# liangheming/simple_pose

Measured on AMD Instinct MI355X. Metric: images/sec fwd+decode, ResNet50-DConv 256x192 bs=128, higher is better.
Workload: dtype f32; 1 GPU; ResNet50-DConv 256x192 bs=128 per GPU, fp32 forward (NCHW in -> heat maps) + GaussTaylor decode, eval-mode BN, conditioned random weights; images_per_gpu=128, global_batch=128, parallelism=replicas x1 (no collective), ranks=1 process(es), one per GPU, launch=stream launches, tile_table=profiles/r06_dconv_f32_tiles.json, batches_in_flight=2, decode=in line, HSA_ENABLE_IPC_MODE_LEGACY=0

## Files before the change

include/simple_pose_hip.h:

```cpp
#ifndef SIMPLE_POSE_HIP_H
#define SIMPLE_POSE_HIP_H

#include <stdint.h>

#ifdef __cplusplus
extern "C" {
#endif

#define SP_OK 0
#define SP_EINVAL (-1)
#define SP_ELAUNCH (-2)

#define SP_ABI_VERSION 36

#define SP_CONV_RELU 0x1u
#define SP_CONV_OUT_NCHW 0x2u
#define SP_CONV_PIXEL_SHUFFLE 0x4u
#define SP_CONV_OUT_F32 0x10u
#define SP_CONV_BN_Y_MASK 0x20u
#define SP_CONV_BF16 0x8u
#define SP_CONV_HARDSWISH 0x40u
#define SP_CONV_OUT_SLICE 0x80u

typedef struct sp_conv_desc {
// ... 1 lines not shown
    int32_t grid_h, grid_w;
    int32_t c_out;
    int32_t n_pad;
    int32_t taps_h, taps_w;
    int32_t k_pad;
    int32_t stride;
    int32_t dy0, dy_step, dx0, dx_step;
    int32_t out_h, out_w, out_c;
    int32_t oy_mul, oy_add, ox_mul, ox_add;
    int32_t phases_y, phases_x;
    uint32_t flags;
    int32_t tile_m, tile_n;
    int32_t stride_x;
    int32_t kernel;
    int32_t c_in_group;
} sp_conv_desc;

#define SP_CONV_KERNEL_IGEMM 0
#define SP_CONV_KERNEL_RING 1
#define SP_CONV_KERNEL_RING_LW 3
#define SP_CONV_KERNEL_RING_LW4 4
#define SP_CONV_KERNEL_PW 2

int sp_abi_version(void);
const char* sp_last_error(void);


int sp_nchw_to_nhwc4(const float* x_nchw, float* y_nhwc4, int batch, int channels, int h, int w, void* stream);

int sp_conv2d_fwd(const sp_conv_desc* desc, const void* x, const void* w_packed, const float* scale,
                  const float* shift, const void* residual, void* y, void* stream);

int sp_conv_set_tap_skip(int on);

int sp_conv3x3_direct_ok(const sp_conv_desc* desc);
int sp_conv3x3_direct(const sp_conv_desc* desc, const void* x, const void* w_packed, const float* scale, const float* shift,
                      const void* residual, void* y, void* stream);

int sp_basic_block_c32_ok(const sp_conv_desc* desc);
int sp_basic_block_c32(const sp_conv_desc* desc, const void* x, const void* w1_packed, const float* scale1, const float* shift1,
                       const void* w2_packed, const float* scale2, const float* shift2, void* y, void* stream);

int sp_basic_block_c64_ok(const sp_conv_desc* desc);
int sp_basic_block_c64(const sp_conv_desc* desc, const void* x, const void* w1_packed, const float* scale1, const float* shift1,
                       const void* w2_packed, const float* scale2, const float* shift2, void* y, void* stream);

int sp_dual_pw_bf16_ok(int64_t rows, int c_main, int c_short, int c_out);
int sp_dual_pw_f32_ok(int64_t rows, int c_main, int c_short, int c_out);
int sp_dual_pw_f32(const float* a_main, const float* w_main_packed, const float* scale_main, const float* shift_main, const float* a_short,
                   const float* w_short_packed, const float* scale_short, const float* shift_short, float* y, int64_t rows, int c_main, int c_short,
                   int c_out, int relu, void* stream);
int sp_dual_pw_bf16(const void* a_main, const void* w_main_packed, const float* scale_main, const float* shift_main, const void* a_short,
                    const void* w_short_packed, const float* scale_short, const float* shift_short, void* y, int64_t rows, int c_main, int c_short,
                    int c_out, int relu, void* stream);
int sp_pw_chain_f32_ok(int64_t rows, int c_mid, int c_out, int c_next);
int sp_pw_chain_f32(const float* t, const float* w3_packed, const float* scale3, const float* shift3, const float* residual, float* y,
                    const float* w1_packed, const float* scale1, const float* shift1, float* t_next, int64_t rows, int c_mid, int c_out, int c_next,
                    void* stream);
int sp_bottleneck_c64_ok(const sp_conv_desc* desc);
int sp_bottleneck_c64(const sp_conv_desc* desc, const void* x, const void* w1_packed, const float* scale1, const float* shift1,
                      const void* w2_packed, const float* scale2, const float* shift2, const void* w3_packed, const float* scale3,
                      const float* shift3, void* y, void* stream);

int sp_stem7_pool_ok(int batch, int h, int w);
int sp_stem7_pool(const float* x, const void* w_packed, int k_pad, const float* scale, const float* shift, void* y, int bf16,
                  int batch, int h, int w, void* stream);
// ... 547 lines not shown
```

simple_pose_amd/_lib.py:

```python
from __future__ import annotations

import ctypes
import os
from ctypes import c_double, c_float, c_int, c_int32, c_int64, c_uint32, c_void_p

from .build import LIB_PATH as _DEFAULT_LIB_PATH

LIB_PATH = os.environ.get("SIMPLE_POSE_HIP_LIB", _DEFAULT_LIB_PATH)

SP_CONV_RELU = 0x1
SP_CONV_OUT_NCHW = 0x2
SP_CONV_PIXEL_SHUFFLE = 0x4
SP_CONV_BF16 = 0x8
SP_CONV_OUT_F32 = 0x10
SP_CONV_BN_Y_MASK = 0x20
SP_CONV_HARDSWISH = 0x40
SP_CONV_OUT_SLICE = 0x80
SP_LETTERBOX_FOCUS, SP_LETTERBOX_U8 = 0, 1
SP_YOLO_NMS_MAX_CANDIDATES, SP_YOLO_NMS_MAX_DET = 32768, 1024
SP_COCO_MAX_JOINTS, SP_COCO_MAX_GT_PER_IMAGE, SP_COCO_MAX_DT_PER_IMAGE, SP_COCO_MAX_DETS = 64, 128, 2048, 32
SP_COCO_DT_XY_F64, SP_COCO_DT_SCORE_F64, SP_COCO_GT_CROWD, SP_COCO_GT_IGNORE = 1, 2, 1, 2
CONV_TILES =((128, 128), (64, 128), (128, 64), (64, 64), (256, 64), (128, 32))
ABI_VERSION = 36
SP_CONV_KERNEL_IGEMM, SP_CONV_KERNEL_RING, SP_CONV_KERNEL_PW, SP_CONV_KERNEL_RING_LW, SP_CONV_KERNEL_RING_LW4 = 0, 1, 2, 3, 4
# ... 104 lines not shown


SP_HEAT_ALPHA_CONSTANT, SP_HEAT_ALPHA_VALUE = 0, 1
SP_HEAT_ALPHAS = {"constant": SP_HEAT_ALPHA_CONSTANT, "value": SP_HEAT_ALPHA_VALUE}
SP_HEAT_MAX_MAP = 256

class TileRef(ctypes.Structure):
    _fields_ = [("data", ctypes.c_uint64), ("h", c_int32), ("w", c_int32), ("pitch", c_int32), ("new_h", c_int32), ("new_w", c_int32),
                ("top", c_int32), ("left", c_int32), ("ratio", c_float), ("x0", c_int32), ("y0", c_int32), ("image", c_int32),
                ("slot", c_int32)]


SP_TILE_MAX_TILES, SP_TILE_MAX_PASSES = 64, 65


class YuvRef(ctypes.Structure):
    _fields_ = [("y", ctypes.c_uint64), ("u", ctypes.c_uint64), ("v", ctypes.c_uint64), ("bgr", ctypes.c_uint64), ("h", c_int32), ("w", c_int32),
                ("pitch_y", c_int32), ("pitch_c", c_int32), ("pitch_bgr", c_int32), ("format", c_int32), ("matrix", c_int32), ("range", c_int32)]


assert ctypes.sizeof(YuvRef) == 64
SP_YUV_NV12, SP_YUV_I420 = 0, 1
SP_YUV_BT601, SP_YUV_BT709 = 0, 1
SP_YUV_LIMITED, SP_YUV_FULL = 0, 1
SP_TILE_IOU, SP_TILE_IOS = 0, 1

_P = c_void_p
SYMBOLS = {
    "sp_abi_version": (c_int, []),
    "sp_last_error": (ctypes.c_char_p, []),
    "sp_nchw_to_nhwc4": (c_int, [_P, _P, c_int, c_int, c_int, c_int, _P]),
    "sp_conv2d_fwd": (c_int, [ctypes.POINTER(ConvDesc), _P, _P, _P, _P, _P, _P, _P]),
    "sp_conv_set_tap_skip": (c_int, [c_int]),
    "sp_conv2d_ring_ok": (c_int, [ctypes.POINTER(ConvDesc)]),
    "sp_conv2d_kernel_name": (c_int, [ctypes.POINTER(ConvDesc), c_int, c_int, ctypes.c_char_p, c_int]),
    "sp_conv2d_default_tile": (c_int, [ctypes.POINTER(ConvDesc), ctypes.POINTER(c_int), ctypes.POINTER(c_int)]),
    "sp_maxpool3x3s2_nhwc": (c_int, [_P, _P, c_int, c_int, c_int, c_int, _P]),
    "sp_pixel_shuffle2_nhwc": (c_int, [_P, _P, c_int, c_int, c_int, c_int, _P]),
    "sp_global_avg_pool_nhwc": (c_int, [_P, _P, c_int, c_int, c_int, _P]),
    "sp_se_gate_add_relu_nhwc": (c_int, [_P, _P, _P, _P, c_int, c_int, c_int, _P]),
    "sp_upsample_add_nhwc": (c_int, [_P, _P, _P, c_int, c_int, c_int, c_int, c_int, c_int, _P]),
    "sp_nchw_to_nhwc8_bf16": (c_int, [_P, _P, c_int, c_int, c_int, c_int, _P]),
    "sp_maxpool3x3s2_nhwc_bf16": (c_int, [_P, _P, c_int, c_int, c_int, c_int, _P]),
    "sp_pixel_shuffle2_nhwc_bf16": (c_int, [_P, _P, c_int, c_int, c_int, c_int, _P]),
    "sp_upsample_add_nhwc_bf16": (c_int, [_P, _P, _P, c_int, c_int, c_int, c_int, c_int, c_int, _P]),
    "sp_global_avg_pool_nhwc_bf16": (c_int, [_P, _P, c_int, c_int, c_int, _P]),
    "sp_se_gate_add_relu_nhwc_bf16": (c_int, [_P, _P, _P, _P, c_int, c_int, c_int, _P]),
    "sp_heat_map_to_axis": (c_int, [_P, c_int, c_int, c_int, c_int, _P, _P, _P]),
    "sp_decode_gauss_taylor": (c_int, [_P, _P, c_int, c_int, c_int, c_int, c_int, _P, _P, _P]),
    "sp_decode_basic": (c_int, [_P, _P, c_int, c_int, c_int, c_int, _P, _P, _P]),
    "sp_heat_map_acc": (c_int, [_P, _P, _P, c_int, c_int, c_int, c_int, c_float, c_float, _P, _P]),
    "sp_u8hwc_bgr_to_nchw_f32": (c_int, [_P, _P, c_int, c_int, c_int, ctypes.POINTER(c_float), _P]),
    "sp_encode_gauss_refine": (c_int, [_P, c_int, c_int, c_int, c_int, c_float, _P, _P, _P]),
    "sp_encode_gauss_basic": (c_int, [_P, c_int, c_int, c_int, c_int, c_float, c_int, _P, _P, _P]),
    "sp_bn_train_stats_nhwc": (c_int, [_P, c_int, c_int64, c_int, c_float, c_float, _P, _P, _P, _P, _P, _P]),
    "sp_bn_apply_maxpool_nhwc": (c_int, [_P, c_int, _P, _P, _P, _P, _P, _P, c_int, c_int, c_int, c_int, _P]),
    "sp_bn_maxpool_bwd_nhwc": (c_int, [_P, c_int, _P, _P, _P, _P, _P, _P, c_int, c_int, c_int, c_int, _P, _P, _P, _P, _P]),
    "sp_bn_apply_nhwc": (c_int, [_P, c_int, _P, _P, _P, _P, _P, _P, c_int64, c_int, c_int, _P, _P]),
    "sp_bn_train_partial_nhwc": (c_int, [_P, c_int, c_int64, c_int, _P, _P, _P]),
    "sp_bn_train_finalize": (c_int, [_P, c_int64, c_int, c_float, c_float, _P, _P, _P, _P, _P]),
    "sp_bn_apply_sums_nhwc": (c_int, [_P, c_int, _P, c_int64, c_float, c_float, _P, _P, _P, _P, c_int64, c_int, c_int, _P, _P, _P, _P, _P]),
    "sp_bn_bwd_sums_from_conv2": (c_int, [_P, _P, c_int, c_int, c_int, _P, _P, _P, _P, _P]),
    "sp_bn_train_bwd_reduce_nhwc": (c_int, [_P, c_int, _P, _P, _P, _P, c_int64, c_int, _P, _P, _P, _P]),
    "sp_bn_train_bwd_apply_nhwc": (c_int, [_P, c_int, _P, _P, _P, _P, _P, _P, _P, c_int64, c_int64, c_int, _P, _P, c_int, _P]),
    "sp_bn_train_bwd_nhwc": (c_int, [_P, c_int, _P, _P, _P, _P, _P, c_int64, c_int, _P, _P, _P, _P, c_int, _P, _P]),
    "sp_channel_sum_nchw": (c_int, [_P, c_int, c_int, c_int, _P, _P]),
# ... 132 lines not shown
    "sp_yuv420_to_bgr_images_u8c3": (c_int, [_P, c_int, c_int, c_int, _P]),
    "sp_bgr_to_yuv420_images_u8c3": (c_int, [_P, c_int, c_int, c_int, _P]),
    "sp_yuv420_wide_path": (c_int, [_P, _P, _P, _P, c_int, c_int, c_int, c_int]),
}

_lib = None


def lib():
    global _lib
    if _lib is None:
        if not os.path.isfile(LIB_PATH):
            raise HipLibraryError(
                f"{LIB_PATH} is missing: build it with `python -m simple_pose_amd.build` (hipcc, gfx950). "
                "simple_pose_amd has no CPU/torch fallback.")
        import torch

        handle = ctypes.CDLL(LIB_PATH)
        for name, (res, args) in SYMBOLS.items():
            fn = getattr(handle, name)
            fn.restype, fn.argtypes = res, args
        if handle.sp_abi_version() != ABI_VERSION:
            raise HipLibraryError(f"ABI mismatch: library {handle.sp_abi_version()} vs binding {ABI_VERSION}")
        _lib = handle
    return _lib


def conv_kernel_name(desc, has_residual: bool = False, variant: int = 0) -> str:
    buf = ctypes.create_string_buffer(256)
    check(lib().sp_conv2d_kernel_name(desc, int(has_residual), variant, buf, 256), "sp_conv2d_kernel_name")
    return buf.value.decode()


def check(rc: int, what: str = ""):
    if rc != 0:
        msg = lib().sp_last_error().decode("utf-8", "replace")
        err = HipLibraryError(f"{what or 'libsimple_pose_hip'} failed (code {rc}): {msg}")
        err.code = rc
        raise err


def ptr(t):
    return None if t is None else t.data_ptr()


import threading

_pin = threading.local()


def _device_index(device) -> int:
    if device is None:
        import torch
        return torch.cuda.current_device()
    if isinstance(device, int):
        return device
    idx = getattr(device, "index", None)
    if idx is None:
        import torch
        return torch.cuda.current_device()
    return idx


def pin_stream(pin):
    prev = getattr(_pin, "value", None)
    _pin.value = pin
# ... 35 lines not shown
```

simple_pose_amd/csrc/conv_igemm.hip:

```cpp
#include "sp_common.h"
#include <stdlib.h>
#include <type_traits>

#ifdef SP_DIAG
__device__ unsigned long long sp_dbg[4096 * 4 * 12];
extern "C" int sp_debug_read(unsigned long long* dst, int n) {
    return (int)hipMemcpyFromSymbol(dst, HIP_SYMBOL(sp_dbg), sizeof(unsigned long long) * n, 0, hipMemcpyDeviceToHost);
}
extern "C" int sp_debug_clear() {
    static unsigned long long z[4096 * 4 * 12];
    return (int)hipMemcpyToSymbol(HIP_SYMBOL(sp_dbg), z, sizeof(z), 0, hipMemcpyHostToDevice);
}
#define SP_STAMP_ALWAYS(var)                                                                \
    unsigned long long var;                                                                 \
    __builtin_amdgcn_sched_barrier(0);                                                      \
    asm volatile("s_memtime %0\n\ts_waitcnt lgkmcnt(0)" : "=s"(var)::"memory");           \
    __builtin_amdgcn_sched_barrier(0);
#ifdef SP_DIAG_LIGHT
#define SP_STAMP(var) unsigned long long var = 0;
#else
#define SP_STAMP(var) SP_STAMP_ALWAYS(var)
#endif
#else
#define SP_STAMP(var)
// ... 30 lines not shown
    const float* binvstd;
    int bz_bytes;
    const void* bz2;
    const float* bmean2;
    const float* binvstd2;
    float* stats_q2;
    struct PhaseGeo { const void* w; int taps_h, taps_w, k_pad, dy0, dx0, oy_add, ox_add, pad_; } ph[4];
    int ph_n;
    int c_in_g;
    const float* abn_mean;
    const float* abn_invstd;
    const float* abn_gamma;
    const float* abn_beta;
    void* abn_y;
    unsigned char* abn_mask;
    int batch;
};

constexpr int BK = 32;

__device__ __forceinline__ float hardswish(float v) {
#pragma clang fp contract(off)
    return v * fminf(fmaxf(v + 3.f, 0.f), 6.f) / 6.f;
}

__device__ __forceinline__ int swz(int row, int chunk) { return row * BK + ((chunk ^ ((row >> 1) & 7)) << 2); }


__device__ __forceinline__ float abn_elem(float v, float mu, float is, float g, float b) {
#pragma clang fp contract(off)
    return (v - mu) * is * g + b;
}

template <int BM, int BN, int WR, int WC, bool UNIFORM_TAP, bool BF16, bool OUT16, bool STATS, bool DEEP, bool BSTATS, bool ABN, bool SKIP = false>
__device__ __forceinline__ void conv_igemm_body(const ConvArgs& p) {
    static_assert(!ABN || (UNIFORM_TAP && BF16 && OUT16 && STATS && !DEEP && !BSTATS), "ABN: the bf16 train-mode forward of a 1x1 conv");
    static_assert(!SKIP || (UNIFORM_TAP && !BF16 && !OUT16 && !STATS && !DEEP && !BSTATS && !ABN), "SKIP: the plain fp32 inference instantiation");
    constexpr int ES = BF16 ? 2 : 4;
    constexpr int EPC = 16 / ES;
    constexpr int BKE = 128 / ES;
    constexpr int ESO = OUT16 ? 2 : 4;
    static_assert(BF16 || !OUT16, "bf16 output needs bf16 inputs");
    static_assert(WR * WC == 4, "4 waves per workgroup");
    constexpr int WM = BM / WR, WN = BN / WC;
    constexpr int TM = WM / 32, TN = WN / 32;
    constexpr int A_CH = BM / 32, B_CH = BN / 32;
    static_assert(TM >= 1 && TN >= 1, "wave tile must hold at least one 32x32 MFMA tile");

#ifdef SP_DIAG
    SP_STAMP_ALWAYS(t_entry)
#endif
#ifdef SP_DIAG
    unsigned long long rt_entry;
    asm volatile("s_memrealtime %0\n\ts_waitcnt lgkmcnt(0)" : "=s"(rt_entry)::"memory");
#endif
    extern __shared__ __attribute__((aligned(16))) float smem[];
    float* As = smem;
    float* Bs = smem + 2 * BM * BK;
    int* rowtab = reinterpret_cast<int*>(smem + 2 * (BM + BN) * BK);

    const int tid = threadIdx.x;
    const int lane = tid & 63;
    const int wave = __builtin_amdgcn_readfirstlane(tid >> 6);
    const int wr = wave / WC, wc = wave % WC;

    const int nwg = p.tiles_m * p.tiles_n;
    int t;
    {
        const int orig = blockIdx.x;
        const int xcd = orig & 7, q = nwg >> 3, r = nwg & 7;
        t = (xcd < r ? xcd * (q + 1) : r * (q + 1) + (xcd - r) * q) + (orig >> 3);
    }
    const int tn = t % p.tiles_n, tm = t / p.tiles_n;
    int tm_rows = tm;
    if constexpr (SKIP) {
        const int Q = p.tiles_m >> 3, R = p.tiles_m & 7;
        int x, i;
        if (tm < R * (Q + 1)) { x = tm / (Q + 1); i = tm - x * (Q + 1); }
        else { const int u = tm - R * (Q + 1); x = u / Q; i = u - x * Q; x += R; }
        tm_rows = i * 8 + x;
    }
    const int m0 = tm_rows * BM, n0 = tn * BN;

    const int phase = blockIdx.y;
    const int py = phase / p.phases_x, px = phase % p.phases_x;
    int dy0 = p.dy0 + py, dx0 = p.dx0 + px;
    int oy_add = p.oy_add + py, ox_add = p.ox_add + px;
    int taps_h = p.taps_h, taps_w = p.taps_w, k_pad = p.k_pad, w_bytes = p.w_bytes;
    const char* __restrict__ wp = reinterpret_cast<const char*>(p.w) + (size_t)phase * p.n_pad * p.k_pad * ES;
    if (p.ph_n) {
        const ConvArgs::PhaseGeo& g = p.ph[phase];
        dy0 = g.dy0; dx0 = g.dx0; oy_add = g.oy_add; ox_add = g.ox_add;
// ... 206 lines not shown
            acc[i][n] = __builtin_amdgcn_mfma_f32_32x32x2f32(fa[slot][i][s], fb[slot][n][s], acc[i][n], 0, 0, 0);
    };
#define SP_SB() __builtin_amdgcn_sched_barrier(0)

    tile_taps(0);
#pragma unroll
    for (int i = 0; i < A_CH; ++i) load_a(i, I0{});
#pragma unroll
    for (int i = 0; i < B_CH; ++i) load_b(i, I0{});
    if constexpr (PF > 1) {
        auto request = [&](auto j_tag) {
            constexpr int J = decltype(j_tag)::value;
            if (J < nk) {
                tile_taps(J);
#pragma unroll
                for (int i = 0; i < A_CH; ++i) load_a(i, j_tag);
#pragma unroll
                for (int i = 0; i < B_CH; ++i) load_b(i, j_tag);
            }
        };
        request(std::integral_constant<int, 1>{});
        if constexpr (PF == 4) { request(std::integral_constant<int, 2>{}); request(std::integral_constant<int, 3>{}); }
    }
#pragma unroll
    for (int o = 0; o < NOPS; ++o) store_piece(0, o, I0{});
    __syncthreads();
    read_frags(As + (wr * WM) * BK, Bs + (wc * WN) * BK, 0, 0);

#ifdef SP_DIAG
    unsigned long long dg[8] = {0, 0, 0, 0, 0, 0, 0, 0};
#endif
    auto k_tile = [&](int kt, auto more_tag) {
        constexpr bool MORE = decltype(more_tag)::value;
        const int cur = kt & 1;
        const float* a = As + cur * BM * BK + (wr * WM) * BK;
        const float* b = Bs + cur * BN * BK + (wc * WN) * BK;
        const float* an = As + (cur ^ 1) * BM * BK + (wr * WM) * BK;
        const float* bn = Bs + (cur ^ 1) * BN * BK + (wc * WN) * BK;
        SP_STAMP(s0)
        read_frags(a, b, 1, 1);
        if (MORE) tile_taps(kt + 1);
        SP_SB();
#pragma unroll
        for (int q = 0; q < NM; ++q) {
            mfma_q(0, q);
            if (MORE) {
#pragma unroll
                for (int o = (q * NOPS) / NM; o < ((q + 1) * NOPS) / NM; ++o) {
                    if (o < A_CH) load_a(o, I0{}); else load_b(o - A_CH, I0{});
                }
            }
            SP_SB();
        }
        SP_STAMP(s1)
        read_frags(a, b, 2, 0);
#pragma unroll
        for (int q = 0; q < NM; ++q) mfma_q(1, q);
        SP_SB();
        SP_STAMP(s2)
        read_frags(a, b, 3, 1);
#pragma unroll
        for (int q = 0; q < NM; ++q) mfma_q(0, q);
        SP_SB();
        SP_STAMP(s3)
        SP_STAMP(s3w)
        constexpr int H3 = NM / 2;
        if constexpr (H3 == 0) {
            if (MORE) {
#pragma unroll
                for (int o = 0; o < NOPS; ++o) store_piece(cur ^ 1, o, I0{});
            }
        } else {
#pragma unroll
            for (int q = 0; q < H3; ++q) {
                mfma_q(1, q);
                if (MORE) {
#pragma unroll
                    for (int o = (q * NOPS) / H3; o < ((q + 1) * NOPS) / H3; ++o) store_piece(cur ^ 1, o, I0{});
                }
                SP_SB();
            }
        }
        SP_STAMP(s4)
        if (MORE) {
            __syncthreads();
        }
        SP_STAMP(s5)
        if (MORE) {
            read_frags(an, bn, 0, 0);
            SP_SB();
        }
#pragma unroll
        for (int q = NM / 2; q < NM; ++q) mfma_q(1, q);
        SP_SB();
#ifdef SP_DIAG
        SP_STAMP(s6)
        dg[0] += s1 - s0; dg[1] += s2 - s1; dg[2] += s3 - s2; dg[3] += s3w - s3; dg[4] += s4 - s3w; dg[5] += s5 - s4; dg[6] += s6 - s5; dg[7] += 1;
#endif
    };
#ifdef SP_DIAG
    SP_STAMP_ALWAYS(t_loop0)
#endif
    if constexpr (PF == 1) {
        for (int kt = 0; kt + 1 < nk; ++kt) k_tile(kt, std::true_type{});
        k_tile(nk - 1, std::false_type{});
    } else {
        auto k_tile_pf = [&](int kt, auto slot_tag, auto load_tag, auto store_tag) {
            constexpr int S = decltype(slot_tag)::value, SN = (S + 1) % PF;
            constexpr bool LOAD = decltype(load_tag)::value, STORE = decltype(store_tag)::value;
            const int cur = kt & 1;
            const float* a = As + cur * BM * BK + (wr * WM) * BK;
// ... 51 lines not shown
        int kt = 0;
        for (; kt + PF < nk; kt += PF) {
            k_tile_pf(kt, std::integral_constant<int, 0>{}, std::true_type{}, std::true_type{});
            k_tile_pf(kt + 1, std::integral_constant<int, 1 % PF>{}, std::true_type{}, std::true_type{});
            if constexpr (PF == 4) {
                k_tile_pf(kt + 2, std::integral_constant<int, 2 % PF>{}, std::true_type{}, std::true_type{});
                k_tile_pf(kt + 3, std::integral_constant<int, 3 % PF>{}, std::true_type{}, std::true_type{});
            }
        }
        if constexpr (PF == 2) {
            k_tile_pf(kt, std::integral_constant<int, 0>{}, std::false_type{}, std::true_type{});
            k_tile_pf(kt + 1, std::integral_constant<int, 1 % PF>{}, std::false_type{}, std::false_type{});
        } else {
            k_tile_pf(kt, std::integral_constant<int, 0>{}, std::false_type{}, std::true_type{});
            k_tile_pf(kt + 1, std::integral_constant<int, 1 % PF>{}, std::false_type{}, std::true_type{});
            k_tile_pf(kt + 2, std::integral_constant<int, 2 % PF>{}, std::false_type{}, std::true_type{});
            k_tile_pf(kt + 3, std::integral_constant<int, 3 % PF>{}, std::false_type{}, std::false_type{});
        }
    }
#ifdef SP_DIAG
    SP_STAMP_ALWAYS(t_loop1)
#endif
    __syncthreads();
#undef SP_SB

    const bool nchw = p.flags & SP_CONV_OUT_NCHW;
    const bool pshuf = p.flags & SP_CONV_PIXEL_SHUFFLE;
    const bool relu = p.flags & SP_CONV_RELU;
    const bool hsw = (!BF16 && !STATS && !BSTATS) && (p.flags & SP_CONV_HARDSWISH);
    const int hw_out = p.out_h * p.out_w;
    const __amdgpu_buffer_rsrc_t yr = __builtin_amdgcn_make_buffer_rsrc(p.y, (short)0, p.y_bytes, 0x00020000);
    const __amdgpu_buffer_rsrc_t rr = __builtin_amdgcn_make_buffer_rsrc(const_cast<void*>(p.res ? p.res : p.y), (short)0, p.y_bytes, 0x00020000);
    if (!nchw && (p.c_out % (16 / ESO)) == 0) {
        static_assert(BM * BN <= 2 * (BM + BN) * BK, "transpose area must fit in the staging buffers");
        float* tr = smem + wave * (WM * WN);
#pragma unroll
        for (int i = 0; i < TM; ++i)
#pragma unroll
            for (int n = 0; n < TN; ++n)
#pragma unroll
                for (int r = 0; r < 16; ++r)
                    tr[(i * 32 + (r & 3) + 8 * (r >> 2) + 4 * fh) * WN + n * 32 + fr] = acc[i][n][r];
        constexpr int CPL = 16 / ESO;
        constexpr int CPR = WN / CPL;
        constexpr int RPI = 64 / CPR;
        constexpr int NIT = WM / RPI;
        const int chunk = lane % CPR, rsub = lane / CPR;
        const int col = n0 + wc * WN + chunk * CPL;
        const bool col_ok = col < p.c_out;
        float sc[CPL], sh[CPL];
#pragma unroll
        for (int e = 0; e < CPL; ++e) { sc[e] = 1.f; sh[e] = 0.f; }
        if (col_ok) {
#pragma unroll
            for (int e4 = 0; e4 < CPL / 4; ++e4) {
                if (p.scale) { const f32x4 t = *reinterpret_cast<const f32x4*>(p.scale + col + 4 * e4); sc[4 * e4] = t[0]; sc[4 * e4 + 1] = t[1]; sc[4 * e4 + 2] = t[2]; sc[4 * e4 + 3] = t[3]; }
                if (p.shift) { const f32x4 t = *reinterpret_cast<const f32x4*>(p.shift + col + 4 * e4); sh[4 * e4] = t[0]; sh[4 * e4 + 1] = t[1]; sh[4 * e4 + 2] = t[2]; sh[4 * e4 + 3] = t[3]; }
            }
        }
        int col_off = col;
        if (pshuf) {
            const int sub = col / p.out_c, c = col - sub * p.out_c;
            col_off = ((sub >> 1) * p.out_w + (sub & 1)) * p.out_c + c;
        }
        unsigned off[NIT];
#pragma unroll
        for (int it = 0; it < NIT; ++it) {
            const int ro = rowtab[(wr * WM + it * RPI + rsub) * 4 + 3];
            off[it] = (col_ok && ro >= 0) ? (unsigned)((ro + col_off) * ESO) : OOB;
        }
        static_assert(!(STATS && BSTATS) && (!BSTATS || !OUT16 || BF16), "BSTATS: fp32 gradients, or bf16 gradients beside bf16 activations");
        float st_s[(STATS || BSTATS) ? CPL : 1], st_q[(STATS || BSTATS) ? CPL : 1];
        float b_mu[BSTATS ? CPL : 1], b_is[BSTATS ? CPL : 1];
        float st_q2[BSTATS ? CPL : 1], b_mu2[BSTATS ? CPL : 1], b_is2[BSTATS ? CPL : 1];
        if constexpr (STATS || BSTATS) {
#pragma unroll
            for (int e = 0; e < CPL; ++e) { st_s[e] = 0.f; st_q[e] = 0.f; }
        }
        if constexpr (BSTATS) {
#pragma unroll
            for (int e = 0; e < CPL; ++e) { b_mu[e] = 0.f; b_is[e] = 0.f; st_q2[e] = 0.f; b_mu2[e] = 0.f; b_is2[e] = 0.f; }
            if (col_ok) {
#pragma unroll
                for (int e4 = 0; e4 < CPL / 4; ++e4) {
                    const f32x4 m4 = *reinterpret_cast<const f32x4*>(p.bmean + col + 4 * e4), i4 = *reinterpret_cast<const f32x4*>(p.binvstd + col + 4 * e4);
#pragma unroll
                    for (int e = 0; e < 4; ++e) { b_mu[4 * e4 + e] = m4[e]; b_is[4 * e4 + e] = i4[e]; }
                    if (p.bz2) {
                        const f32x4 m2 = *reinterpret_cast<const f32x4*>(p.bmean2 + col + 4 * e4), i2 = *reinterpret_cast<const f32x4*>(p.binvstd2 + col + 4 * e4);
#pragma unroll
                        for (int e = 0; e < 4; ++e) { b_mu2[4 * e4 + e] = m2[e]; b_is2[4 * e4 + e] = i2[e]; }
                    }
                }
            }
        }
        const bool by_mask = BSTATS && OUT16 && (p.flags & SP_CONV_BN_Y_MASK);
        const __amdgpu_buffer_rsrc_t byr = __builtin_amdgcn_make_buffer_rsrc(const_cast<void*>(BSTATS ? p.by : p.y), (short)0,
                                                                             BSTATS ? (by_mask ? p.bz_bytes >> 4 : p.bz_bytes) : 0, 0x00020000);
        const __amdgpu_buffer_rsrc_t bzr = __builtin_amdgcn_make_buffer_rsrc(const_cast<void*>(BSTATS ? p.bz : p.y), (short)0, BSTATS ? p.bz_bytes : 0, 0x00020000);
        const __amdgpu_buffer_rsrc_t bz2r = __builtin_amdgcn_make_buffer_rsrc(const_cast<void*>((BSTATS && p.bz2) ? p.bz2 : p.y), (short)0, (BSTATS && p.bz2) ? p.bz_bytes : 0, 0x00020000);
        u32x4 rv[NIT];
        if (p.res) {
#pragma unroll
            for (int it = 0; it < NIT; ++it) rv[it] = __builtin_amdgcn_raw_buffer_load_b128(rr, off[it], 0, 0);
        }
#pragma unroll
        for (int it = 0; it < NIT; ++it) {
            float v[CPL];
#pragma unroll
            for (int e4 = 0; e4 < CPL / 4; ++e4) {
                const f32x4 t = *reinterpret_cast<const f32x4*>(tr + (it * RPI + rsub) * WN + chunk * CPL + 4 * e4);
                v[4 * e4] = t[0]; v[4 * e4 + 1] = t[1]; v[4 * e4 + 2] = t[2]; v[4 * e4 + 3] = t[3];
            }
#pragma unroll
            for (int e = 0; e < CPL; ++e) v[e] = v[e] * sc[e] + sh[e];
            if (hsw) {
#pragma unroll
                for (int e = 0; e < CPL; ++e) v[e] = hardswish(v[e]);
            }
            if (p.res) {
                if constexpr (OUT16) {
                    const bf16x8 r8 = __builtin_bit_cast(bf16x8, rv[it]);
                    if (p.res_mask) {
                        const __amdgpu_buffer_rsrc_t rmr = __builtin_amdgcn_make_buffer_rsrc(const_cast<unsigned char*>(p.res_mask), (short)0, p.y_bytes >> 4, 0x00020000);
                        const unsigned m = __builtin_amdgcn_raw_buffer_load_b8(rmr, off[it] == OOB ? OOB : off[it] >> 4, 0, 0);
#pragma unroll
                        for (int e = 0; e < 8; ++e) v[e] += ((m >> e) & 1u) ? (float)r8[e] : 0.f;
                    } else {
#pragma unroll
                        for (int e = 0; e < 8; ++e) v[e] += (float)r8[e];
                    }
                } else {
                    const f32x4 r4 = __builtin_bit_cast(f32x4, rv[it]);
#pragma unroll
                    for (int e = 0; e < 4; ++e) v[e] += r4[e];
                }
            }
            if (relu) {
#pragma unroll
                for (int e = 0; e < CPL; ++e) v[e] = v[e] > 0.f ? v[e] : 0.f;
            }
            u32x4 o;
            if constexpr (OUT16) {
                bf16x8 o8;
// ... 161 lines not shown
                    }
                }
            }
        }
    }
#ifdef SP_DIAG
    SP_STAMP_ALWAYS(t_issued)
    asm volatile("s_waitcnt vmcnt(0)" ::: "memory");
    SP_STAMP_ALWAYS(t_end)
    unsigned long long rt_end;
    asm volatile("s_memrealtime %0\n\ts_waitcnt lgkmcnt(0)" : "=s"(rt_end)::"memory");
    if (lane == 0 && blockIdx.y == 0) {
        unsigned long long* o = sp_dbg + ((blockIdx.x & 4095) * 4 + wave) * 12;
#pragma unroll
        for (int q = 0; q < 8; ++q) o[q] = dg[q];
        o[8] = t_loop0 - t_entry; o[9] = t_loop1 - t_loop0; o[10] = t_end - t_loop1; o[11] = t_end - t_issued; o[7] = (rt_end - rt_entry) | (rt_entry << 32);
    }
#endif
}

template <int BM, int BN, int WR, int WC, bool UNIFORM_TAP, bool BF16, bool OUT16, bool STATS = false, bool DEEP = false, bool BSTATS = false>
__global__ __launch_bounds__(256, (BM * BN > 128 * 128) ? 1 : 2) void conv_igemm_kernel(const ConvArgs p) {
    conv_igemm_body<BM, BN, WR, WC, UNIFORM_TAP, BF16, OUT16, STATS, DEEP, BSTATS, false>(p);
}

template <int BM, int BN, int WR, int WC>
__global__ __launch_bounds__(256, (BM * BN > 128 * 128) ? 1 : 2) void conv_igemm_abn_kernel(const ConvArgs p) {
    conv_igemm_body<BM, BN, WR, WC, true, true, true, true, false, false, true>(p);
}

template <int BM, int BN, int WR, int WC>
__global__ __launch_bounds__(256, (BM * BN > 128 * 128) ? 1 : 2) void conv_igemm_tapskip_kernel(const ConvArgs p) {
    conv_igemm_body<BM, BN, WR, WC, true, false, false, false, false, false, false, true>(p);
}

template <int BM, int BN, int WR, int WC, bool BF16, bool OUT16, bool STATS, bool DEEP = false, bool BSTATS = false>
int launch_t(const ConvArgs& a, int phases, bool uniform, hipStream_t stream) {
    if constexpr (!DEEP && BF16) {
        constexpr int pf = BM * BN <= 64 * 64 ? 4 : 2;
        int nk = a.k_pad / 64;
        bool whole = nk % pf == 0;
        if (a.ph_n) {
            nk = 0;
            whole = true;
            for (int i = 0; i < a.ph_n; ++i) {
                const int n = a.ph[i].k_pad / 64;
                whole = whole && n % pf == 0;
                nk = n > nk ? n : nk;
            }
        }
        if (whole && nk >= (BM * BN <= 64 * 64 ? 12 : 32))
            return launch_t<BM, BN, WR, WC, BF16, OUT16, STATS, true, BSTATS>(a, phases, uniform, stream);
    }
    if (sp_name_query_active()) {
        auto t = [](bool v) { return v ? "true" : "false"; };
        sp_name_query_set("conv_igemm_kernel<%d, %d, %d, %d, %s, %s, %s, %s, %s, %s>", BM, BN, WR, WC, t(uniform), t(BF16), t(OUT16), t(STATS), t(DEEP), t(BSTATS));
        return SP_OK;
    }
    ConvArgs p = a;
    p.tiles_m = (a.M + BM - 1) / BM;
    p.tiles_n = a.n_pad / BN;
    const size_t lds = (size_t)2 * (BM + BN) * BK * sizeof(float) + (size_t)BM * 4 * sizeof(int) +
                       ((STATS || BSTATS) ? (size_t)3 * WR * BN * sizeof(float) : 0);
    dim3 grid(p.tiles_m * p.tiles_n, phases, 1), block(256, 1, 1);
    if (sp_reserve_lds<&conv_igemm_kernel<BM, BN, WR, WC, true, BF16, OUT16, STATS, DEEP, BSTATS>>((int)lds, "conv_igemm") ||
        sp_reserve_lds<&conv_igemm_kernel<BM, BN, WR, WC, false, BF16, OUT16, STATS, DEEP, BSTATS>>((int)lds, "conv_igemm"))
// ... 7 lines not shown

template <int BM, int BN, int WR, int WC>
int launch_abn(const ConvArgs& a, hipStream_t stream) {
    if (sp_name_query_active()) {
        sp_name_query_set("conv_igemm_abn_kernel<%d, %d, %d, %d>", BM, BN, WR, WC);
        return SP_OK;
    }
    ConvArgs p = a;
    p.tiles_m = (a.M + BM - 1) / BM;
    p.tiles_n = a.n_pad / BN;
    const size_t lds = (size_t)2 * (BM + BN) * BK * sizeof(float) + (size_t)BM * 4 * sizeof(int) + (size_t)3 * WR * BN * sizeof(float) +
                       (size_t)a.c_in * 4 * sizeof(float);
    const size_t lds_max = (size_t)2 * (BM + BN) * BK * sizeof(float) + (size_t)BM * 4 * sizeof(int) + (size_t)3 * WR * BN * sizeof(float) + 512 * 16;
    if (sp_reserve_lds<&conv_igemm_abn_kernel<BM, BN, WR, WC>>((int)lds_max, "conv_igemm_abn")) return SP_ELAUNCH;
    hipLaunchKernelGGL((conv_igemm_abn_kernel<BM, BN, WR, WC>), dim3(p.tiles_m * p.tiles_n, 1, 1), dim3(256, 1, 1), lds, stream, p);
    return sp_check_launch("conv_igemm_abn_kernel");
}

template <int BM, int BN, int WR, int WC>
int launch_tapskip(const ConvArgs& a, int phases, hipStream_t stream) {
    if (sp_name_query_active()) {
        sp_name_query_set("conv_igemm_tapskip_kernel<%d, %d, %d, %d>", BM, BN, WR, WC);
        return SP_OK;
    }
    ConvArgs p = a;
    p.tiles_m = (a.M + BM - 1) / BM;
    p.tiles_n = a.n_pad / BN;
    const size_t lds = (size_t)2 * (BM + BN) * BK * sizeof(float) + (size_t)BM * 4 * sizeof(int);
    if (sp_reserve_lds<&conv_igemm_tapskip_kernel<BM, BN, WR, WC>>((int)lds, "conv_igemm_tapskip")) return SP_ELAUNCH;
    hipLaunchKernelGGL((conv_igemm_tapskip_kernel<BM, BN, WR, WC>), dim3(p.tiles_m * p.tiles_n, phases, 1), dim3(256, 1, 1), lds, stream, p);
    return sp_check_launch("conv_igemm_tapskip_kernel");
}

template <int BM, int BN, int WR, int WC>
int launch(const ConvArgs& a, int phases, bool uniform, bool tap_skip, hipStream_t stream) {
    if (tap_skip && a.batch >= BM / 2) return launch_tapskip<BM, BN, WR, WC>(a, phases, stream);
    if (a.abn_mean) return launch_abn<BM, BN, WR, WC>(a, stream);
    if (a.bz) {
        if ((a.flags & SP_CONV_BF16) && !(a.flags & SP_CONV_OUT_F32)) return launch_t<BM, BN, WR, WC, true, true, false, false, true>(a, phases, uniform, stream);
        if (a.flags & SP_CONV_BF16) return launch_t<BM, BN, WR, WC, true, false, false, false, true>(a, phases, uniform, stream);
        return launch_t<BM, BN, WR, WC, false, false, false, false, true>(a, phases, uniform, stream);
    }
    if (a.stats_s) {
        if (a.flags & SP_CONV_BF16) return launch_t<BM, BN, WR, WC, true, true, true>(a, phases, uniform, stream);
        return launch_t<BM, BN, WR, WC, false, false, true>(a, phases, uniform, stream);
    }
    if (a.flags & SP_CONV_BF16) {
        if (a.flags & SP_CONV_OUT_F32) return launch_t<BM, BN, WR, WC, true, false, false>(a, phases, uniform, stream);
        return launch_t<BM, BN, WR, WC, true, true, false>(a, phases, uniform, stream);
    }
    return launch_t<BM, BN, WR, WC, false, false, false>(a, phases, uniform, stream);
}

}

extern "C" int sp_conv2d_default_tile(const sp_conv_desc* d, int* tile_m, int* tile_n);
int sp_conv_ring_launch(const sp_conv_desc* d, const void* x, const void* w_packed, const float* scale, const float* shift,
                        const void* residual, void* y, void* stream);
int sp_conv_pw_launch(const sp_conv_desc* d, const void* x, const void* w_packed, const float* scale, const float* shift,
                      const void* residual, void* y, void* stream);

static int tile_rows_per_block(int, int) { return 1; }

static int g_tap_skip = -1;
static bool tap_skip_enabled() {
    if (g_tap_skip < 0) { const char* e = getenv("SP_CONV_TAP_SKIP"); g_tap_skip = (e && atoi(e) == 0) ? 0 : 1; }
    return g_tap_skip != 0;
}
extern "C" int sp_conv_set_tap_skip(int on) {
    g_tap_skip = on ? 1 : 0;
    return SP_OK;
}

struct BnBwdSrc { const void* y; const void* z; const float* mean; const float* invstd; const void* z2; const float* mean2; const float* invstd2; float* q2;
                  const void* res_mask = nullptr; };

struct PhaseSet { const sp_conv_desc* descs; const void* const* w; int n; };
struct AbnSrc { const float* mean; const float* invstd; const float* gamma; const float* beta; void* y; unsigned char* mask; };

static int conv_fwd_impl(const sp_conv_desc* d, const void* x, const void* w_packed, const float* scale, const float* shift,
                         const void* residual, void* y, float* stats_s, float* stats_q, int stats_rows_capacity, void* stream,
                         const BnBwdSrc* bsrc = nullptr, const PhaseSet* phs = nullptr, const AbnSrc* abn = nullptr) {
    SP_REQUIRE(d && x && w_packed && y, "sp_conv2d_fwd: null pointer");
    SP_REQUIRE(d->batch > 0 && d->in_h > 0 && d->in_w > 0 && d->grid_h > 0 && d->grid_w > 0 && d->c_out > 0,
               "sp_conv2d_fwd: non-positive dimension");
    const bool bf16 = d->flags & SP_CONV_BF16;
    const int es = bf16 ? 2 : 4, epc = 16 / es, bke = 128 / es;
    SP_REQUIRE(d->c_in > 0 && d->c_in % epc == 0, "sp_conv2d_fwd: c_in=%d must be a positive multiple of %d", d->c_in, epc);
    SP_REQUIRE(d->taps_h > 0 && d->taps_w > 0 && d->stride > 0 && d->stride_x >= 0, "sp_conv2d_fwd: bad taps/stride");
    const int cg = d->c_in_group > 0 ? d->c_in_group : d->c_in;
    SP_REQUIRE(d->k_pad % bke == 0 && d->k_pad >= d->taps_h * d->taps_w * cg,
               "sp_conv2d_fwd: k_pad=%d must be a multiple of %d and >= taps*c_in=%d", d->k_pad, bke,
               d->taps_h * d->taps_w * cg);
    if (d->c_in_group > 0) {
        SP_REQUIRE(d->c_in_group % bke == 0 && d->c_in % d->c_in_group == 0 && d->c_out == d->c_in && d->n_pad == d->c_out &&
                       d->tile_n == d->c_in_group && d->kernel == SP_CONV_KERNEL_IGEMM && d->phases_y == 1 && d->phases_x == 1 && !bsrc && !stats_s && !phs &&
                       !(d->flags & SP_CONV_PIXEL_SHUFFLE) && d->taps_h * d->taps_w <= 32,
                   "sp_conv2d_fwd: grouped launch needs c_in_group = tile_n (a multiple of %d dividing c_in), c_out == c_in == n_pad, the implicit-GEMM "
                   "kernel, one phase, no statistics epilogue (c_in_group %d, tile_n %d, c_in %d, c_out %d)", bke, d->c_in_group, d->tile_n, d->c_in, d->c_out);
    }
    SP_REQUIRE(d->n_pad % 32 == 0 && d->n_pad >= d->c_out, "sp_conv2d_fwd: n_pad=%d must be a multiple of 32 >= c_out=%d",
               d->n_pad, d->c_out);
    const bool uniform = (cg % bke == 0) && d->taps_h * d->taps_w <= 32;
// ... 148 lines not shown
    SP_REQUIRE(d && buf && cap > 0, "sp_conv2d_kernel_name: null pointer");
    SP_REQUIRE(variant >= 0 && variant <= 6, "sp_conv2d_kernel_name: variant %d", variant);
    void* const dummy = reinterpret_cast<void*>(16);
    if (variant >= 4) {
        void* const dummy2 = reinterpret_cast<void*>(32);
        sp_name_query_begin();
        const int rcb = variant == 4 ? sp_basic_block_c32(d, dummy, dummy, nullptr, nullptr, dummy, nullptr, nullptr, dummy2, nullptr)
                      : variant == 6 ? sp_basic_block_c64(d, dummy, dummy, nullptr, nullptr, dummy, nullptr, nullptr, dummy2, nullptr)
                                     : sp_bottleneck_c64(d, dummy, dummy, nullptr, nullptr, dummy, nullptr, nullptr, dummy, nullptr, nullptr, dummy2, nullptr);
        const char* nameb = sp_name_query_end();
        if (rcb != SP_OK) return rcb;
        snprintf(buf, (size_t)cap, "%s", nameb);
        return SP_OK;
    }
    if (variant == 3) {
        sp_name_query_begin();
        const int rc3 = sp_conv3x3_direct(d, dummy, dummy, nullptr, nullptr, has_residual ? dummy : nullptr, dummy, nullptr);
        const char* name3 = sp_name_query_end();
        if (rc3 != SP_OK) return rc3;
        snprintf(buf, (size_t)cap, "%s", name3);
        return SP_OK;
    }
    float* const fdummy = reinterpret_cast<float*>(16);
    const BnBwdSrc src = {dummy, dummy, fdummy, fdummy, nullptr, nullptr, nullptr, nullptr};
    sp_name_query_begin();
    const int rc = conv_fwd_impl(d, dummy, dummy, nullptr, nullptr, has_residual ? dummy : nullptr, dummy, variant ? fdummy : nullptr,
                                 variant ? fdummy : nullptr, 1 << 30, nullptr, variant == 2 ? &src : nullptr);
    const char* name = sp_name_query_end();
    if (rc != SP_OK) return rc;
    snprintf(buf, (size_t)cap, "%s", name);
    return SP_OK;
}

extern "C" int sp_conv2d_bn_stats_rows(const sp_conv_desc* d, int* rows) {
    if (!d || !rows) { sp_set_error("sp_conv2d_bn_stats_rows: null pointer"); return SP_EINVAL; }
    int bm = d->tile_m, bn = d->tile_n;
    if (bm == 0 && bn == 0) sp_conv2d_default_tile(d, &bm, &bn);
    SP_REQUIRE(bm > 0 && bn > 0, "sp_conv2d_bn_stats_rows: bad tile");
    const long long M = (long long)d->batch * d->grid_h * d->grid_w;
    *rows = (int)((long long)d->phases_y * d->phases_x * ((M + bm - 1) / bm) * tile_rows_per_block(bm, bn));
    return SP_OK;
}

extern "C" int sp_conv2d_fwd_bn_stats(const sp_conv_desc* d, const void* x, const void* w_packed, void* y, float* stats_sum,
                                      float* stats_sumsq, int stats_rows_capacity, void* stream) {
    SP_REQUIRE(stats_sum && stats_sumsq, "sp_conv2d_fwd_bn_stats: null statistics pointer");
    return conv_fwd_impl(d, x, w_packed, nullptr, nullptr, nullptr, y, stats_sum, stats_sumsq, stats_rows_capacity, stream);
}

extern "C" int sp_conv2d_fwd_bn_stats_abn(const sp_conv_desc* d, const void* z_in, const float* in_mean, const float* in_invstd, const float* in_gamma,
                                          const float* in_beta, void* y_in, void* relu_mask_in, const void* w_packed, void* y, float* stats_sum,
                                          float* stats_sumsq, int stats_rows_capacity, void* stream) {
    SP_REQUIRE(stats_sum && stats_sumsq, "sp_conv2d_fwd_bn_stats_abn: null statistics pointer");
    const AbnSrc abn = {in_mean, in_invstd, in_gamma, in_beta, y_in, reinterpret_cast<unsigned char*>(relu_mask_in)};
    return conv_fwd_impl(d, z_in, w_packed, nullptr, nullptr, nullptr, y, stats_sum, stats_sumsq, stats_rows_capacity, stream, nullptr, nullptr, &abn);
}

extern "C" int sp_conv2d_dgrad_bn_bwd_stats(const sp_conv_desc* d, const void* dz, const void* w_packed, const void* accumulate, void* dx,
                                           const void* bn_y, const void* bn_z, const float* bn_mean, const float* bn_invstd,
                                           float* sum_g, float* sum_g_xhat, int stats_rows_capacity, void* stream) {
    const BnBwdSrc src = {bn_y, bn_z, bn_mean, bn_invstd, nullptr, nullptr, nullptr, nullptr};
    return conv_fwd_impl(d, dz, w_packed, nullptr, nullptr, accumulate, dx, sum_g, sum_g_xhat, stats_rows_capacity, stream, &src);
}

extern "C" int sp_conv2d_dgrad_bn_bwd_stats2(const sp_conv_desc* d, const void* dz, const void* w_packed, const void* accumulate, void* dx,
                                            const void* bn_y, const void* bn_z, const float* bn_mean, const float* bn_invstd,
// ... 59 lines not shown
```

Baseline: 11780 images/s.

## Add single-buffered LDS variant of fp32 128x128 igemm conv for higher occupancy

Adds a SINGLE template mode to the implicit-GEMM conv body that uses one LDS staging buffer instead of two, with an extra barrier before overwriting the tile. The output transpose is done in 32-row slices so it fits the smaller LDS area. Halving LDS lets launch bounds ask for 3 resident workgroups instead of 2. The variant is enabled by default for 128x128 fp32 uniform and tap-skip convs. The cost is losing the double-buffered overlap of global loads with MFMA, plus extra barriers.

Measured after the change: 11940 images/s, median of 6. 1.4% higher.

```diff
diff --git a/include/simple_pose_hip.h b/include/simple_pose_hip.h
--- a/include/simple_pose_hip.h
+++ b/include/simple_pose_hip.h
@@ -57,6 +57,10 @@
                   const float* shift, const void* residual, void* y, void* stream);
 
 int sp_conv_set_tap_skip(int on);
+
+int sp_conv_set_single_stage(int on);
+int sp_conv2d_single_stage(const sp_conv_desc* desc, int has_residual);
+int sp_conv_igemm_resident_workgroups(int which, int* workgroups, int* lds_bytes);
 
 int sp_conv3x3_direct_ok(const sp_conv_desc* desc);
 int sp_conv3x3_direct(const sp_conv_desc* desc, const void* x, const void* w_packed, const float* scale, const float* shift,
diff --git a/simple_pose_amd/_lib.py b/simple_pose_amd/_lib.py
--- a/simple_pose_amd/_lib.py
+++ b/simple_pose_amd/_lib.py
@@ -160,6 +160,9 @@
     "sp_nchw_to_nhwc4": (c_int, [_P, _P, c_int, c_int, c_int, c_int, _P]),
     "sp_conv2d_fwd": (c_int, [ctypes.POINTER(ConvDesc), _P, _P, _P, _P, _P, _P, _P]),
     "sp_conv_set_tap_skip": (c_int, [c_int]),
+    "sp_conv_set_single_stage": (c_int, [c_int]),
+    "sp_conv2d_single_stage": (c_int, [ctypes.POINTER(ConvDesc), c_int]),
+    "sp_conv_igemm_resident_workgroups": (c_int, [c_int, ctypes.POINTER(c_int), ctypes.POINTER(c_int)]),
     "sp_conv2d_ring_ok": (c_int, [ctypes.POINTER(ConvDesc)]),
     "sp_conv2d_kernel_name": (c_int, [ctypes.POINTER(ConvDesc), c_int, c_int, ctypes.c_char_p, c_int]),
     "sp_conv2d_default_tile": (c_int, [ctypes.POINTER(ConvDesc), ctypes.POINTER(c_int), ctypes.POINTER(c_int)]),
@@ -358,6 +361,10 @@
     return buf.value.decode()
 
 
+def conv_single_stage(desc, has_residual: bool = False) -> bool:
+    return bool(lib().sp_conv2d_single_stage(desc, int(has_residual)))
+
+
 def check(rc: int, what: str = ""):
     if rc != 0:
         msg = lib().sp_last_error().decode("utf-8", "replace")
diff --git a/simple_pose_amd/csrc/conv_igemm.hip b/simple_pose_amd/csrc/conv_igemm.hip
--- a/simple_pose_amd/csrc/conv_igemm.hip
+++ b/simple_pose_amd/csrc/conv_igemm.hip
@@ -86,10 +86,13 @@
     return (v - mu) * is * g + b;
 }
 
-template <int BM, int BN, int WR, int WC, bool UNIFORM_TAP, bool BF16, bool OUT16, bool STATS, bool DEEP, bool BSTATS, bool ABN, bool SKIP = false>
+template <int BM, int BN, int WR, int WC, bool UNIFORM_TAP, bool BF16, bool OUT16, bool STATS, bool DEEP, bool BSTATS, bool ABN, bool SKIP = false,
+          bool SINGLE = false>
 __device__ __forceinline__ void conv_igemm_body(const ConvArgs& p) {
     static_assert(!ABN || (UNIFORM_TAP && BF16 && OUT16 && STATS && !DEEP && !BSTATS), "ABN: the bf16 train-mode forward of a 1x1 conv");
     static_assert(!SKIP || (UNIFORM_TAP && !BF16 && !OUT16 && !STATS && !DEEP && !BSTATS && !ABN), "SKIP: the plain fp32 inference instantiation");
+    static_assert(!SINGLE || (UNIFORM_TAP && !BF16 && !OUT16 && !STATS && !DEEP && !BSTATS && !ABN), "SINGLE: the plain fp32 inference instantiation");
+    constexpr int NBUF = SINGLE ? 1 : 2;
     constexpr int ES = BF16 ? 2 : 4;
     constexpr int EPC = 16 / ES;
     constexpr int BKE = 128 / ES;
@@ -110,8 +113,8 @@
 #endif
     extern __shared__ __attribute__((aligned(16))) float smem[];
     float* As = smem;
-    float* Bs = smem + 2 * BM * BK;
-    int* rowtab = reinterpret_cast<int*>(smem + 2 * (BM + BN) * BK);
+    float* Bs = smem + NBUF * BM * BK;
+    int* rowtab = reinterpret_cast<int*>(smem + NBUF * (BM + BN) * BK);
 
     const int tid = threadIdx.x;
     const int lane = tid & 63;
@@ -384,11 +387,11 @@
 #endif
     auto k_tile = [&](int kt, auto more_tag) {
         constexpr bool MORE = decltype(more_tag)::value;
-        const int cur = kt & 1;
+        const int cur = SINGLE ? 0 : kt & 1, nxt = SINGLE ? 0 : cur ^ 1;
         const float* a = As + cur * BM * BK + (wr * WM) * BK;
         const float* b = Bs + cur * BN * BK + (wc * WN) * BK;
-        const float* an = As + (cur ^ 1) * BM * BK + (wr * WM) * BK;
-        const float* bn = Bs + (cur ^ 1) * BN * BK + (wc * WN) * BK;
+        const float* an = As + nxt * BM * BK + (wr * WM) * BK;
+        const float* bn = Bs + nxt * BN * BK + (wc * WN) * BK;
         SP_STAMP(s0)
         read_frags(a, b, 1, 1);
         if (MORE) tile_taps(kt + 1);
@@ -415,12 +418,15 @@
         for (int q = 0; q < NM; ++q) mfma_q(0, q);
         SP_SB();
         SP_STAMP(s3)
+        if constexpr (SINGLE) {
+            if (MORE) __syncthreads();
+        }
         SP_STAMP(s3w)
         constexpr int H3 = NM / 2;
         if constexpr (H3 == 0) {
             if (MORE) {
 #pragma unroll
-                for (int o = 0; o < NOPS; ++o) store_piece(cur ^ 1, o, I0{});
+                for (int o = 0; o < NOPS; ++o) store_piece(nxt, o, I0{});
             }
         } else {
 #pragma unroll
@@ -428,7 +434,7 @@
                 mfma_q(1, q);
                 if (MORE) {
 #pragma unroll
-                    for (int o = (q * NOPS) / H3; o < ((q + 1) * NOPS) / H3; ++o) store_piece(cur ^ 1, o, I0{});
+                    for (int o = (q * NOPS) / H3; o < ((q + 1) * NOPS) / H3; ++o) store_piece(nxt, o, I0{});
                 }
                 SP_SB();
             }
@@ -546,15 +552,17 @@
     const __amdgpu_buffer_rsrc_t yr = __builtin_amdgcn_make_buffer_rsrc(p.y, (short)0, p.y_bytes, 0x00020000);
     const __amdgpu_buffer_rsrc_t rr = __builtin_amdgcn_make_buffer_rsrc(const_cast<void*>(p.res ? p.res : p.y), (short)0, p.y_bytes, 0x00020000);
     if (!nchw && (p.c_out % (16 / ESO)) == 0) {
-        static_assert(BM * BN <= 2 * (BM + BN) * BK, "transpose area must fit in the staging buffers");
-        float* tr = smem + wave * (WM * WN);
-#pragma unroll
-        for (int i = 0; i < TM; ++i)
-#pragma unroll
-            for (int n = 0; n < TN; ++n)
-#pragma unroll
-                for (int r = 0; r < 16; ++r)
-                    tr[(i * 32 + (r & 3) + 8 * (r >> 2) + 4 * fh) * WN + n * 32 + fr] = acc[i][n][r];
+        static_assert(SINGLE ? BM * BN / TM <= (BM + BN) * BK : BM * BN <= 2 * (BM + BN) * BK, "transpose area must fit in the staging buffers");
+        float* tr = smem + wave * (SINGLE ? 32 * WN : WM * WN);
+        if constexpr (!SINGLE) {
+#pragma unroll
+            for (int i = 0; i < TM; ++i)
+#pragma unroll
+                for (int n = 0; n < TN; ++n)
+#pragma unroll
+                    for (int r = 0; r < 16; ++r)
+                        tr[(i * 32 + (r & 3) + 8 * (r >> 2) + 4 * fh) * WN + n * 32 + fr] = acc[i][n][r];
+        }
         constexpr int CPL = 16 / ESO;
         constexpr int CPR = WN / CPL;
         constexpr int RPI = 64 / CPR;
@@ -621,9 +629,22 @@
 #pragma unroll
         for (int it = 0; it < NIT; ++it) {
             float v[CPL];
+            if constexpr (SINGLE) {
+                static_assert(32 % RPI == 0, "a wave-instruction stays inside one 32-row group");
+                if ((it * RPI) % 32 == 0) {
+                    __builtin_amdgcn_wave_barrier();
+#pragma unroll
+                    for (int n = 0; n < TN; ++n)
+#pragma unroll
+                        for (int r = 0; r < 16; ++r)
+                            tr[((r & 3) + 8 * (r >> 2) + 4 * fh) * WN + n * 32 + fr] = acc[(it * RPI) / 32][n][r];
+                    __builtin_amdgcn_wave_barrier();
+                }
+            }
 #pragma unroll
             for (int e4 = 0; e4 < CPL / 4; ++e4) {
-                const f32x4 t = *reinterpret_cast<const f32x4*>(tr + (it * RPI + rsub) * WN + chunk * CPL + 4 * e4);
+                const f32x4 t = SINGLE ? *reinterpret_cast<const f32x4*>(tr + ((it * RPI) % 32 + rsub) * WN + chunk * CPL + 4 * e4)
+                                       : *reinterpret_cast<const f32x4*>(tr + (it * RPI + rsub) * WN + chunk * CPL + 4 * e4);
                 v[4 * e4] = t[0]; v[4 * e4 + 1] = t[1]; v[4 * e4 + 2] = t[2]; v[4 * e4 + 3] = t[3];
             }
 #pragma unroll
@@ -851,6 +872,16 @@
 template <int BM, int BN, int WR, int WC>
 __global__ __launch_bounds__(256, (BM * BN > 128 * 128) ? 1 : 2) void conv_igemm_tapskip_kernel(const ConvArgs p) {
     conv_igemm_body<BM, BN, WR, WC, true, false, false, false, false, false, false, true>(p);
+}
+
+template <int BM, int BN, int WR, int WC>
+__global__ __launch_bounds__(256, 3) void conv_igemm_single_kernel(const ConvArgs p) {
+    conv_igemm_body<BM, BN, WR, WC, true, false, false, false, false, false, false, false, true>(p);
+}
+
+template <int BM, int BN, int WR, int WC>
+__global__ __launch_bounds__(256, 3) void conv_igemm_tapskip_single_kernel(const ConvArgs p) {
+    conv_igemm_body<BM, BN, WR, WC, true, false, false, false, false, false, false, true, true>(p);
 }
 
 template <int BM, int BN, int WR, int WC, bool BF16, bool OUT16, bool STATS, bool DEEP = false, bool BSTATS = false>
@@ -924,9 +955,46 @@
     return sp_check_launch("conv_igemm_tapskip_kernel");
 }
 
+int g_single_stage = -1;
+thread_local int g_single_taken = 0;
+bool single_stage_enabled() {
+    if (g_single_stage < 0) { const char* e = getenv("SP_CONV_SINGLE_STAGE"); g_single_stage = (e && atoi(e) == 0) ? 0 : 1; }
+    return g_single_stage != 0;
+}
+
+template <int BM, int BN, int WR, int WC, bool SKIP>
+int launch_single(const ConvArgs& a, int phases, hipStream_t stream) {
+    if (sp_name_query_active()) {
+        g_single_taken = 1;
+        if (SKIP) sp_name_query_set("conv_igemm_tapskip_kernel<%d, %d, %d, %d>", BM, BN, WR, WC);
+        else sp_name_query_set("conv_igemm_kernel<%d, %d, %d, %d, true, false, false, false, false, false>", BM, BN, WR, WC);
+        return SP_OK;
+    }
+    ConvArgs p = a;
+    p.tiles_m = (a.M + BM - 1) / BM;
+    p.tiles_n = a.n_pad / BN;
+    const size_t lds = (size_t)(BM + BN) * BK * sizeof(float) + (size_t)BM * 4 * sizeof(int);
+    const dim3 grid(p.tiles_m * p.tiles_n, phases, 1), block(256, 1, 1);
+    if constexpr (SKIP) {
+        if (sp_reserve_lds<&conv_igemm_tapskip_single_kernel<BM, BN, WR, WC>>((int)lds, "conv_igemm_tapskip_single")) return SP_ELAUNCH;
+        hipLaunchKernelGGL((conv_igemm_tapskip_single_kernel<BM, BN, WR, WC>), grid, block, lds, stream, p);
+        return sp_check_launch("conv_igemm_tapskip_single_kernel");
+    } else {
+        if (sp_reserve_lds<&conv_igemm_single_kernel<BM, BN, WR, WC>>((int)lds, "conv_igemm_single")) return SP_ELAUNCH;
+        hipLaunchKernelGGL((conv_igemm_single_kernel<BM, BN, WR, WC>), grid, block, lds, stream, p);
+        return sp_check_launch("conv_igemm_single_kernel");
+    }
+}
+
 template <int BM, int BN, int WR, int WC>
 int launch(const ConvArgs& a, int phases, bool uniform, bool tap_skip, hipStream_t stream) {
-    if (tap_skip && a.batch >= BM / 2) return launch_tapskip<BM, BN, WR, WC>(a, phases, stream);
+    constexpr bool HAS_SINGLE = BM == 128 && BN == 128;
+    if (tap_skip && a.batch >= BM / 2) {
+        if constexpr (HAS_SINGLE) {
+            if (single_stage_enabled()) return launch_single<BM, BN, WR, WC, true>(a, phases, stream);
+        }
+        return launch_tapskip<BM, BN, WR, WC>(a, phases, stream);
+    }
     if (a.abn_mean) return launch_abn<BM, BN, WR, WC>(a, stream);
     if (a.bz) {
         if ((a.flags & SP_CONV_BF16) && !(a.flags & SP_CONV_OUT_F32)) return launch_t<BM, BN, WR, WC, true, true, false, false, true>(a, phases, uniform, stream);
@@ -941,6 +1009,9 @@
         if (a.flags & SP_CONV_OUT_F32) return launch_t<BM, BN, WR, WC, true, false, false>(a, phases, uniform, stream);
         return launch_t<BM, BN, WR, WC, true, true, false>(a, phases, uniform, stream);
     }
+    if constexpr (HAS_SINGLE) {
+        if (uniform && !a.c_in_g && !a.ph_n && single_stage_enabled()) return launch_single<BM, BN, WR, WC, false>(a, phases, stream);
+    }
     return launch_t<BM, BN, WR, WC, false, false, false>(a, phases, uniform, stream);
 }
 
@@ -961,6 +1032,11 @@
 }
 extern "C" int sp_conv_set_tap_skip(int on) {
     g_tap_skip = on ? 1 : 0;
+    return SP_OK;
+}
+
+extern "C" int sp_conv_set_single_stage(int on) {
+    g_single_stage = on ? 1 : 0;
     return SP_OK;
 }
 
@@ -1175,6 +1251,44 @@
     return SP_OK;
 }
 
+extern "C" int sp_conv2d_single_stage(const sp_conv_desc* d, int has_residual) {
+    if (!d) { sp_set_error("sp_conv2d_single_stage: null pointer"); return 0; }
+    void* const dummy = reinterpret_cast<void*>(16);
+    sp_name_query_begin();
+    g_single_taken = 0;
+    const int rc = conv_fwd_impl(d, dummy, dummy, nullptr, nullptr, has_residual ? dummy : nullptr, dummy, nullptr, nullptr, 0, nullptr);
+    sp_name_query_end();
+    const int taken = g_single_taken;
+    g_single_taken = 0;
+    return rc == SP_OK ? taken : 0;
+}
+
+extern "C" int sp_conv_igemm_resident_workgroups(int which, int* workgroups, int* lds_bytes) {
+    SP_REQUIRE(lds_bytes && which >= 0 && which <= 3, "sp_conv_igemm_resident_workgroups: which = 0..3 and a result pointer");
+    const int rowtab = 128 * 4 * (int)sizeof(int);
+    const int lds = (which >= 2 ? 1 : 2) * (128 + 128) * BK * (int)sizeof(float) + rowtab;
+    *lds_bytes = lds;
+    if (!workgroups) return SP_OK;
+    const void* f = nullptr;
+    int rc = SP_OK;
+    switch (which) {
+        case 0: f = reinterpret_cast<const void*>(&conv_igemm_kernel<128, 128, 2, 2, true, false, false, false, false, false>);
+                rc = sp_reserve_lds<&conv_igemm_kernel<128, 128, 2, 2, true, false, false, false, false, false>>(lds, "conv_igemm"); break;
+        case 1: f = reinterpret_cast<const void*>(&conv_igemm_tapskip_kernel<128, 128, 2, 2>);
+                rc = sp_reserve_lds<&conv_igemm_tapskip_kernel<128, 128, 2, 2>>(lds, "conv_igemm_tapskip"); break;
+        case 2: f = reinterpret_cast<const void*>(&conv_igemm_single_kernel<128, 128, 2, 2>);
+                rc = sp_reserve_lds<&conv_igemm_single_kernel<128, 128, 2, 2>>(lds, "conv_igemm_single"); break;
+        default: f = reinterpret_cast<const void*>(&conv_igemm_tapskip_single_kernel<128, 128, 2, 2>);
+                rc = sp_reserve_lds<&conv_igemm_tapskip_single_kernel<128, 128, 2, 2>>(lds, "conv_igemm_tapskip_single"); break;
+    }
+    if (rc) return SP_ELAUNCH;
+    int n = 0;
+    const hipError_t e = hipOccupancyMaxActiveBlocksPerMultiprocessor(&n, f, 256, (size_t)lds);
+    if (e != hipSuccess) { sp_set_error("sp_conv_igemm_resident_workgroups: %s", hipGetErrorString(e)); return SP_ELAUNCH; }
+    *workgroups = n;
+    return SP_OK;
+}
+
 extern "C" int sp_conv2d_bn_stats_rows(const sp_conv_desc* d, int* rows) {
     if (!d || !rows) { sp_set_error("sp_conv2d_bn_stats_rows: null pointer"); return SP_EINVAL; }
     int bm = d->tile_m, bn = d->tile_n;
```
